# jmhb0/view_neti

Hardware: AMD Instinct MI355X
Metric: TI train steps/sec (SD-1.5 512^2 bs=4 per GPU) (higher is better)
Workload: dtype f16; 1 GPU; learnable_mode 0, sd15 shapes, 512x512 fp16, bs=4/GPU, grad_accum 1, full train step (VAE+16xCLIP+UNet fwd/bwd+AdamW); global_batch=4, parallelism=dp1, rccl_ranks=1, hipgraph=True

## Files before the change

### include/vneti.h

```cpp
#ifndef VNETI_H
#define VNETI_H
#include <stddef.h>
#include <stdint.h>

#ifdef __cplusplus
extern "C" {
#endif

#define VNETI_ABI_VERSION 1

int vneti_version(void);
int vneti_precision(void);
int vneti_last_error(char* buf, size_t n);

typedef struct vneti_gemm_desc {
  const void* A;
  const void* B;
  void* C;
  long long lda, ldb, ldc;
  int M, N, K;
  int batch;
  long long strideA, strideB, strideC;
  const float* bias;
  const void* rowadd;
  long long ld_rowadd;
  int rows_per_group;
  const void* resid;
  long long ldr;
  float alpha;
  int act;
  int out_f32;
  int conv_mode;
  int Hi, Wi, Ci, Ho, Wo, stride, pad_t, pad_l, ups;
  long long ldx;
  int tile_hint;
  void* workspace;
  long long workspace_bytes;
  int split_k;
  const void* gate_src;
  long long ld_gate;
  int gate_act;
  void* C2;
  long long ldc2;
  int act2;
  void* gn_sums;
  int gn_hw, gn_cpg, gn_groups, gn_slots;
  int geglu;
  int conv_korder;
} vneti_gemm_desc;

int vneti_gemm_f16(const vneti_gemm_desc* d, void* stream);
int vneti_gemm_select_tile(int M, int N, int batch);
int vneti_gemm_select_split(int M, int N, int K, int batch, int tile_hint, long long workspace_bytes);

int vneti_im2col3x3_small(const void* x, int x_is_f32, long long sb, long long sc, long long sy,
                          long long sx, void* out, int Bn, int C, int Hi, int Wi, int Ho, int Wo,
                          int stride, int pad_t, int pad_l, void* stream);

int vneti_conv3x3_in(const void* x, int x_is_f32, long long sb, long long sc, long long sy, long long sx,
                     const void* w_packed, const float* bias, void* out, long long ldo, int Bn, int C, int H, int W,
                     int Co, void* gn_sums, int gn_groups, int gn_slots, void* stream);

int vneti_transpose_f16(const void* in, long long ld_in, long long stride_in, void* out,
                        long long ld_out, long long stride_out, int rows, int cols, int batch,
                        void* stream);
#define VNETI_TRANSPOSE_MAX 4
typedef struct vneti_transpose_desc {
  const void* inp;
  long long ld_in, stride_in;
  void* out;
  long long ld_out, stride_out;
  int rows, cols, batch, _pad;
} vneti_transpose_desc;
int vneti_transpose_f16_multi(const vneti_transpose_desc* descs, int n, void* stream);

long long vneti_groupnorm_ws_floats(int Bn, int HW, int C, int G);
int vneti_groupnorm_fwd(const void* x, long long ldx, void* y, long long ldy, const float* gamma,
                        const float* beta, float* mean, float* rstd, float* ws, int Bn, int HW,
                        int C, int G, float eps, int silu, void* stream);
int vneti_groupnorm_fwd_sums(const void* x, long long ldx, void* y, long long ldy, const float* gamma,
                             const float* beta, const void* sums, int slots, float* mean, float* rstd,
                             int Bn, int HW, int C, int G, float eps, int silu, void* stream);
int vneti_groupnorm_fwd_2l(const void* x, long long ldx, void* y, long long ldy, const float* gamma,
                           const float* beta, void* sums, int slots, float* mean, float* rstd, int Bn, int HW,
                           int C, int G, float eps, int silu, void* stream);
int vneti_groupnorm_bwd_2l(const void* dy, long long lddy, const void* x, long long ldx, const float* gamma,
                           const float* beta, const float* mean, const float* rstd, void* dx, long long lddx,
                           const void* dx_accum, long long ldacc, void* sums, int slots, float* ws, int Bn,
                           int HW, int C, int G, int silu, void* stream);
int vneti_groupnorm_bwd(const void* dy, long long lddy, const void* x, long long ldx,
                        const float* gamma, const float* beta, const float* mean,
                        const float* rstd, void* dx, long long lddx, const void* dx_accum,
                        long long ldacc, float* ws, int Bn, int HW, int C, int G, int silu,
                        void* stream);

int vneti_layernorm_fwd(const void* x, int x_is_f32, long long ldx, void* y, long long ldy,
                        const float* gamma, const float* beta, float* mean, float* rstd, int rows,
                        int C, float eps, void* stream);
int vneti_layernorm_bwd(const void* dy, int dy_is_f32, long long lddy, const void* x,
                        int x_is_f32, long long ldx, const float* gamma, const float* mean,
                        const float* rstd, void* dx, int dx_is_f32, long long lddx,
                        const void* dx_accum, long long ldacc, void* dx_f16_copy, long long ldcopy,
                        int rows, int C, void* stream);

int vneti_attn_fwd(const void* Q, long long ldq, const void* K, long long ldk, const void* V,
                   long long ldv, void* O, long long ldo, float* lse, int Bn, int H, int Nq,
// ... 159 lines not shown
```

### view_neti_amd/csrc/gemm_conv.hip

```cpp
#include "common.h"
#include "gemm_args.h"
#include "../../include/vneti.h"

namespace {

template <int BM, int BN, int WM, int WN, bool F32OUT, bool DMA, int NSTG = 2, int EPI = 2, bool CONV = true>
__global__ __launch_bounds__((BM / WM) * (BN / WN) * 64) void gemm_kernel(
    const half_t* pA, const half_t* pB, uint32_t p_a_bytes, uint32_t p_b_bytes, int p_lda, int p_ldb, int pM, int pN, int pK,
    int p_tiles_m, int p_tiles_n, int p_split_conv , const GemmArgs gfull) {
  GemmArgs g = gfull;
  g.A = pA;
  g.B = pB;
  g.a_bytes = p_a_bytes;
  g.b_bytes = p_b_bytes;
  g.lda = p_lda;
  g.ldb = p_ldb;
  g.M = pM;
  g.N = pN;
  g.K = pK;
  g.tiles_m = p_tiles_m;
  g.tiles_n = p_tiles_n;
  g.kt_per_split = p_split_conv & 0xffff;
  g.ksplit = (p_split_conv >> 16) & 0xff;
  g.conv_mode = p_split_conv >> 24;
  static_assert(NSTG == 2 || ((NSTG == 3 || NSTG == 4) && DMA), "the LDS rings are LDS-DMA only");
  const half_t* const e_gate = EPI == 2 ? g.gate_src : nullptr;
  half_t* const e_C2 = EPI == 2 ? g.C2 : nullptr;
  const int e_geglu = EPI == 2 ? g.geglu : 0;
  const int e_act = EPI == 2 ? g.act : 0;
  float* const e_gn_sums = EPI >= 1 ? g.gn_sums : nullptr;
  const half_t* const e_rowadd = EPI >= 1 ? g.rowadd : nullptr;
  const int e_conv = CONV ? g.conv_mode : 0;
  constexpr int NWM = BM / WM, NWN = BN / WN;
  constexpr int NT = NWM * NWN * 64;
  constexpr int RSTEP = NT / 8;
  constexpr int A_IT = BM / RSTEP, B_IT = BN / RSTEP;
  constexpr int STAGE_BYTES = (BM + BN) * 128;
  constexpr int CS_LD = F32OUT ? (BN + 4) : (BN + 8);
  constexpr int CS_BYTES = BM * CS_LD * (F32OUT ? 4 : 2);
  constexpr int LDS_BYTES = (NSTG * STAGE_BYTES > CS_BYTES) ? NSTG * STAGE_BYTES : CS_BYTES;
  constexpr int GN_IMG = 5, GN_NG = BN / 4 + 2;
  constexpr int GN_BYTES = (F32OUT || EPI == 0) ? 0 : GN_IMG * GN_NG * 4 * 8;
  __shared__ __attribute__((aligned(16))) char smem[LDS_BYTES + GN_BYTES];

  const int tid = threadIdx.x;
  const int lane = tid & 63;
  const int wave = __builtin_amdgcn_readfirstlane(tid >> 6);
  const int wm0 = (wave / NWN) * WM;
  const int wn0 = (wave % NWN) * WN;

  int nblk = g.tiles_m * g.tiles_n;
  int bid = blockIdx.x;
  {
    int q = nblk >> 3, r = nblk & 7, xcd = bid & 7, idx = bid >> 3;
    bid = (xcd < r ? xcd * (q + 1) : r * (q + 1) + (xcd - r) * q) + idx;
  }
  const int tile_m = bid / g.tiles_n;
  const int tile_n = bid - tile_m * g.tiles_n;
  const int m0 = tile_m * BM;
  const int n0 = tile_n * BN;
  const int bz = blockIdx.y;
  const int kz = blockIdx.z;

  const half_t* Ab = g.A + (long long)bz * g.strideA;
  const half_t* Bb = g.B + (long long)bz * g.strideB;
  __amdgpu_buffer_rsrc_t rsA = vn_make_rsrc(Ab, g.a_bytes);
  __amdgpu_buffer_rsrc_t rsB = vn_make_rsrc(Bb, g.b_bytes);

  const int lrow = tid >> 3;
  const int gchunk = DMA ? ((tid & 7) ^ ((lrow >> 1) & 7)) : (tid & 7);

  const float rcp_hw = CONV ? __builtin_amdgcn_rcpf((float)(g.Ho * g.Wo)) : 0.f, rcp_wo = CONV ? __builtin_amdgcn_rcpf((float)g.Wo) : 0.f;
  int a_off[A_IT];
  int a_py[A_IT], a_px[A_IT], a_bh[A_IT];
#pragma unroll
  for (int i = 0; i < A_IT; ++i) {
    int m = m0 + lrow + RSTEP * i;
    bool ok = m < g.M;
    if (e_conv == 0) {
      a_off[i] = ok ? (int)((long long)m * g.lda * 2) + gchunk * 16 : -1;
      a_py[i] = a_px[i] = a_bh[i] = 0;
    } else {
      int rem, ox;
      const int b = vn_divmod(m, g.Ho * g.Wo, rcp_hw, rem);
      const int oy = vn_divmod(rem, g.Wo, rcp_wo, ox);
      a_bh[i] = ok ? b * g.Hi : -1;
      if (e_conv == 1) {
        a_py[i] = oy * g.stride - g.pad_t;
        a_px[i] = ox * g.stride - g.pad_l;
      } else {
        a_py[i] = oy + g.pad_t;
        a_px[i] = ox + g.pad_l;
      }
      a_off[i] = ((b * g.Hi + a_py[i]) * g.Wi + a_px[i]) * g.ldx2 + gchunk * 16;
    }
  }
  int b_off[B_IT];
#pragma unroll
  for (int i = 0; i < B_IT; ++i) {
    int n = n0 + lrow + RSTEP * i;
    b_off[i] = (n < g.N) ? (int)((long long)n * g.ldb * 2) + gchunk * 16 : -1;
  }

  u32x4 ra[DMA ? 1 : A_IT], rb[DMA ? 1 : B_IT];

  auto a_offset = [&](int i, int k0, int dy, int dx, int tapoff) -> uint32_t {
    if (e_conv == 0) return a_off[i] < 0 ? VN_OOB : (uint32_t)(a_off[i] + k0 * 2);
    bool ok = a_bh[i] >= 0;
    if (e_conv == 1 && !g.ups) {
      int iy = a_py[i] + dy, ix = a_px[i] + dx;
      ok = ok && (unsigned)iy < (unsigned)g.Hi && (unsigned)ix < (unsigned)g.Wi;
      return ok ? (uint32_t)(a_off[i] + tapoff) : VN_OOB;
    }
    int iy, ix;
    if (e_conv == 1) {
// ... 765 lines not shown
  if (cfg == 17 && f32) cfg = 7;
  if ((cfg == 6 || cfg == 7) && !dma) cfg = 4;
  if (cfg >= 10 && !dma) cfg = kTiles[cfg].bm == 128 ? (kTiles[cfg].bn == 128 ? 1 : 2) : 3;
  long long ws_floats = d->workspace ? d->workspace_bytes / 4 : 0;
  int ks = d->split_k;
  if (ks == 0) ks = select_ksplit(d->M, d->N, d->K, batch, cfg, ws_floats);
  if (ks < 1) ks = 1;
  const int nk = d->K / 64;
  if (ks > nk) ks = nk;
  if (ks > 1) {
    VN_REQUIRE(d->workspace && (long long)ks * batch * d->M * d->N <= ws_floats,
               "gemm: split_k=%d needs %lld workspace bytes", ks, (long long)ks * batch * d->M * d->N * 4);
    VN_REQUIRE(batch == 1 || (d->strideC != 0), "gemm: batched split-K needs strideC");
    VN_REQUIRE((long long)batch * d->M * ((d->N + 3) / 4) < 0x7fffffffLL, "gemm: split-K output larger than 2^31 chunks");
    VN_REQUIRE_OUT("gemm split-K workspace", (long long)ks * batch * d->M * d->N * 4);
  }
  if (cfg == 18 && ks > d->Ci / 64) ks = d->Ci / 64;
  g.ksplit = ks;
  g.kt_per_split = cdiv(nk, ks);
  g.ksplit = cdiv(nk, g.kt_per_split);
  VN_REQUIRE(g.ksplit <= 255 && g.kt_per_split <= 0xffff, "gemm: split_k=%d / K=%d out of range", g.ksplit, d->K);
  g.ws = (float*)d->workspace;

#define LAUNCH(BM, BN, WM, WN) \
  return dma ? launch_cfg<BM, BN, WM, WN, true>(g, f32, st) : launch_cfg<BM, BN, WM, WN, false>(g, f32, st)
  switch (cfg) {
    case 1: LAUNCH(128, 128, 64, 64);
    case 2: LAUNCH(128, 64, 64, 32);
    case 3: LAUNCH(64, 64, 32, 32);
    case 4: LAUNCH(256, 128, 64, 64);
    case 6: return launch_cfg_ring<256, 128, 64, 64>(g, f32, st);
    case 7: return launch_cfg_ring<256, 128, 64, 32>(g, f32, st);
    case 8: LAUNCH(256, 128, 64, 32);
    case 9: LAUNCH(128, 128, 64, 32);
    case 10: return launch_cfg_ring<128, 128, 64, 32>(g, f32, st);
    case 11: return launch_cfg_ring<128, 64, 64, 32>(g, f32, st);
    case 12: return launch_cfg_ring<64, 64, 32, 32>(g, f32, st);
    case 13: return launch_cfg_ring<128, 128, 64, 32, 4>(g, f32, st);
    case 14: return launch_cfg_ring<128, 64, 64, 32, 4>(g, f32, st);
    case 15: return launch_cfg_ring<64, 64, 32, 32, 4>(g, f32, st);
    case 16:
    case 17:
    case 18: {
      const int rc = vneti_launch_gemm8(&g, cfg == 16 ? 256 : 128, cfg == 18 ? 1 : 0, st);
      if (rc != VNETI_OK) return rc;
      launch_reduce(g, st);
      return vneti_check_launch("gemm8_kernel");
    }
    default:
      return dma ? launch_cfg_f16<256, 256, 64, 64, true>(g, st) : launch_cfg_f16<256, 256, 64, 64, false>(g, st);
  }
#undef LAUNCH
}
```

### view_neti_amd/engine/step.py

```python
from __future__ import annotations

from functools import partial
from typing import Dict, List, Optional

import torch

from .. import ops
from .. import sd_config as sc
from .graphs import capture_graphs
from .text import MapperState, TextEngine
from .unet import UNetEngine
from .vae import VAEEncoderEngine


def alphas_cumprod(cfg: sc.DDPMConfig) -> torch.Tensor:
    betas = torch.linspace(cfg.beta_start ** 0.5, cfg.beta_end ** 0.5, cfg.num_train_timesteps,
                           dtype=torch.float32) ** 2
    return torch.cumprod(1.0 - betas, dim=0)


class TrainStepEngine:
    def __init__(self, cfg: sc.SDConfig, unet_w: Dict, vae_w: Dict, clip_w: Dict, batch: int, height: int,
                 width: int, mapper_object: Dict[str, torch.Tensor], w_enc_object: torch.Tensor,
                 norm_scale_object: Optional[float], alpha_object: float = 0.2,
                 mapper_view: Optional[Dict[str, torch.Tensor]] = None, w_enc_view: Optional[torch.Tensor] = None,
                 norm_scale_view: Optional[float] = None, alpha_view: float = 0.2, train_view: bool = True,
                 n_view_params: int = 12, lr: float = 1e-3, betas=(0.9, 0.999), adam_eps: float = 1e-8,
                 weight_decay: float = 1e-2, loss_scale: Optional[float] = None, growth_interval: int = 2000,
                 seed: int = 0, world_size: int = 1, device_rng: bool = True, device: str = "cuda",
                 need_backward: bool = True, grad_accum: int = 1, overlap: bool = False,
                 unconstrained_object: bool = False, unconstrained_view: bool = False,
                 nested_dropout_prob: float = 0.0, hidden_object: int = 64,
                 legacy_pe_object: Optional[torch.Tensor] = None, enc_dim_object: int = 64,
                 output_bypass_object: bool = True, output_bypass_view: bool = True, exchange=None,
                 moment_cache_images: int = 0):
        from .text import flatten_mapper_state
        self.cfg = cfg
        self.B, self.H, self.W = batch, height, width
        self.dev = device
        self.world_size = world_size
        self.exchange = exchange
        if world_size > 1 and exchange is None:
            import os
            import torch.distributed as dist
            if os.environ.get("VNETI_RCCL_DIRECT", "1") != "0" and dist.is_initialized() and dist.get_backend() == "nccl":
                from ..parallel import enable_direct_rccl
                try:
                    self.exchange = enable_direct_rccl()
                except RuntimeError as err:
                    if os.environ.get("VNETI_REQUIRE_ONE_GRAPH", "0") == "1":
                        raise
                    import warnings
                    warnings.warn(f"library RCCL communicator unavailable ({err}); using torch.distributed.all_reduce")
        self.device_rng = device_rng
        if loss_scale is None:
            from .. import lib
            loss_scale = 1.0 if lib.precision() == "bf16" else 65536.0
            if lib.precision() == "bf16":
                growth_interval = 0
        self.growth_interval = growth_interval
        nlev = len(cfg.vae.block_out_channels)
        self.h, self.w = height >> (nlev - 1), width >> (nlev - 1)
        Lc = cfg.vae.latent_channels
        D = cfg.clip.hidden_size
        objs = list(mapper_object) if isinstance(mapper_object, (list, tuple)) else [mapper_object]
        flats = [flatten_mapper_state(sd) for sd in objs]
        self.n_objects = len(flats)
        self.n_obj = flats[0].numel()
        assert all(f.numel() == self.n_obj for f in flats), "object mappers must share one architecture"
        flat_v = flatten_mapper_state(mapper_view) if (mapper_view is not None and train_view) else None
        n_all_obj = self.n_obj * self.n_objects
        n = n_all_obj + (flat_v.numel() if flat_v is not None else 0)
        self.params = torch.zeros(n, dtype=torch.float32, device=device)
        self.params[:n_all_obj].copy_(torch.cat(flats))
        if flat_v is not None:
            self.params[n_all_obj:].copy_(flat_v)
        self.grads = torch.zeros_like(self.params)
        self.exp_avg = torch.zeros_like(self.params)
        self.exp_avg_sq = torch.zeros_like(self.params)
        self.n_all_obj = n_all_obj
        self.obj_slot = torch.zeros(1, dtype=torch.int32, device=device)
        self.seg_step = torch.zeros(self.n_objects, dtype=torch.int32, device=device)
        self.active_object = 0
        multi = self.n_objects > 1
        self.rng_state = torch.tensor([seed & 0x7FFFFFFF, 0], dtype=torch.int32, device=device)
        mo = MapperState(self.params[:n_all_obj],
                         w_enc_object.to(device).float().contiguous() if legacy_pe_object is None else None,
                         norm_scale_object, alpha_object, hidden=hidden_object, enc_dim=enc_dim_object,
                         unconstrained=unconstrained_object,
                         nested_dropout_prob=nested_dropout_prob, slot=self.obj_slot if multi else None,
                         slot_stride=self.n_obj if multi else 0,
                         legacy_w_pe=(legacy_pe_object.to(device).float().contiguous()
                                      if legacy_pe_object is not None else None),
                         output_bypass=output_bypass_object)
        mv, gv = None, None
        if mapper_view is not None:
            if flat_v is not None:
                pv, gv = self.params[n_all_obj:], self.grads[n_all_obj:]
            else:
                pv = flatten_mapper_state(mapper_view).to(device)
            mv = MapperState(pv, w_enc_view.to(device).float().contiguous(), norm_scale_view, alpha_view,
                             unconstrained=unconstrained_view,
                             nested_dropout_prob=nested_dropout_prob if flat_v is not None else 0.0,
                             output_bypass=output_bypass_view)
        self.grad_accum = grad_accum
        self.hyper = torch.tensor([lr, betas[0], betas[1], adam_eps, weight_decay, float(world_size * grad_accum)],
                                  dtype=torch.float32, device=device)
        self.scaler = torch.tensor([loss_scale, 0.0, 0.0], dtype=torch.float32, device=device)
        self.opt_step = torch.zeros(1, dtype=torch.int32, device=device)
        self.loss_sum = torch.zeros(1, dtype=torch.float32, device=device)
        self.ac = alphas_cumprod(cfg.ddpm).to(device)
        from ..parallel import shared_picks
        with shared_picks():
            self.unet = UNetEngine(cfg.unet, unet_w, batch, self.h, self.w, cfg.clip.max_positions, device, need_backward)
            self.vae = VAEEncoderEngine(cfg.vae, vae_w, batch, height, width, device)
            self.text = TextEngine(cfg.clip, clip_w, cfg.unet.n_cross_layers, batch, self.unet.timesteps, self.unet.ctx_k,
                                   self.unet.ctx_v, self.unet.dctx_k, self.unet.dctx_v, mo, self.grads[:n_all_obj], mv,
                                   gv, n_view_params, train_view, device, need_backward, rng_state=self.rng_state)
        self.timesteps = self.unet.timesteps
        self.pixel_values = self.vae.x_in
        shape = (batch, Lc, self.h, self.w)
        self.eps = torch.zeros(shape, dtype=torch.float32, device=device)
        self.noise = torch.zeros(shape, dtype=torch.float32, device=device)
        self.latents = torch.zeros(shape, dtype=torch.float32, device=device)
        self.target = torch.zeros(shape, dtype=torch.float32, device=device)
        self.n_cache = int(moment_cache_images)
        if self.n_cache:
            hw2 = self.h * self.w
            self.mcache = torch.zeros(self.n_cache, hw2, 2 * Lc, dtype=self.vae.moments.dtype, device=device)
            self.img_idx = torch.zeros(batch, dtype=torch.int64, device=device)
            self._cached_images = set()
            self._batch_cached = False
            self._batch_images = ()
        self.graph_a_c = self.graph_acc_c = None
        self.eval_out = torch.zeros(batch, dtype=torch.float32, device=device)
        self.eval_ws = torch.zeros(ops.mse_loss_per_sample_ws_floats(batch, self.h * self.w), dtype=torch.float32,
                                   device=device)
        self.graph_eval = None
        from .staging import HostStager
        self.stager = HostStager()
        self.need_backward = need_backward
        self.overlap = overlap
        self.side = torch.cuda.Stream() if overlap else None
        self.graph_a = self.graph_b = self.graph_acc = None
        self.exchange_in_graph = False
        self._reduce_stage = None
        self.last_reduce_bytes = 0
        self.micro = 0
        self._eval_batch = False
        self.n_loss = batch * Lc * self.h * self.w

    def set_batch(self, pixel_values, input_ids, placeholder_object, placeholder_view=None, view_params=None,
                  object_index: int = 0, image_idx=None, for_eval: bool = False):
        if not 0 <= object_index < self.n_objects:
            raise ValueError(f"object_index {object_index} out of range (have {self.n_objects} object mappers)")
        if self.micro != 0 and object_index != self.active_object:
            raise ValueError("the object mapper may not change inside a gradient-accumulation group")
        self.active_object = object_index
        self.obj_slot.fill_(object_index)
        self._eval_batch = bool(for_eval)
        st = self.stager
        st.begin()
        try:
            if self.n_cache and for_eval:
                self._batch_images, self._batch_cached = (), False
            elif self.n_cache:
                if image_idx is None:
# ... 297 lines not shown
```

### view_neti_amd/engine/unet.py

```python
from __future__ import annotations

from functools import partial
from typing import Dict

import torch

from .. import ops, packing
from .. import sd_config as sc
from .schedule import Schedule, T, rup as _rup


class UNetEngine(Schedule):
    def __init__(self, cfg: sc.UNetConfig, weights: Dict[str, torch.Tensor], batch: int, height: int, width: int,
                 ctx_len: int = 77, device: str = "cuda", need_backward: bool = True, autotune: bool = True,
                 fuse_gn: bool = True):
        super().__init__(batch, cfg.norm_num_groups, cfg.norm_eps, device, need_backward)
        self.cfg = cfg
        self.H, self.W = height, width
        self.L = ctx_len
        self.nl = cfg.n_cross_layers
        B, L, Dc = batch, ctx_len, cfg.cross_attention_dim
        self.x_in = self._buf((B, cfg.in_channels, height, width), torch.float32)
        self.timesteps = torch.zeros(B, dtype=torch.int64, device=device)
        self.ctx_k = self._buf((self.nl, B * L, Dc))
        self.ctx_v = self._buf((self.nl, B * L, Dc))
        self.dctx_k = self._buf((self.nl, B * L, Dc))
        self.dctx_v = self._buf((self.nl, B * L, Dc))
        self.pred = self._buf((B * height * width, 8))[:, : cfg.out_channels]
        self.dpred = self._buf((B * height * width, 8), zero=True)[:, : cfg.out_channels]
        self._pack_time_weights(weights)
        self._plan_kv()
        self._build(weights)
        self._kv_fwd_ops()
        if need_backward:
            self._build_backward()
            self._kv_bwd_ops()
        if autotune:
            self.autotune()
        self.bind_workspace()
        self.fuse_gn_stats(fuse=fuse_gn)

    def _pack_time_weights(self, w):
        cfg = self.cfg
        names = [k[: -len("time_emb_proj.weight")] for k in sc.unet_shapes(cfg) if k.endswith("time_emb_proj.weight")]
        self.temb_off = {}
        ws, bs, off = [], [], 0
        for n in names:
            wt = w[n + "time_emb_proj.weight"]
            self.temb_off[n] = (off, wt.shape[0])
            ws.append(wt)
            bs.append(w[n + "time_emb_proj.bias"])
            off += wt.shape[0]
        self.temb_total = off
        self.w_temb_all = self._w16(torch.cat(ws, 0))
        self.b_temb_all = self._w32(torch.cat(bs, 0))
        self.w_t1 = self._w16(w["time_embedding.linear_1.weight"])
        self.b_t1 = self._w32(w["time_embedding.linear_1.bias"])
        self.w_t2 = self._w16(w["time_embedding.linear_2.weight"])
        self.b_t2 = self._w32(w["time_embedding.linear_2.bias"])
        c0, td = cfg.block_out_channels[0], cfg.temb_dim
        self.t_sin = self._buf((self.B, c0))
        self.t_h = self._buf((self.B, td))
        self.t_emb = self._buf((self.B, td))
        self.temb_all = self._buf((self.B, self.temb_total))

    def _time_ops(self):
        f = self.fwd_pre
        f.append(partial(ops.timestep_embedding, self.timesteps, self.t_sin))
        f.append(partial(ops.gemm, self.t_sin, self.w_t1, self.t_h, bias=self.b_t1, act=ops.ACT_SILU, tile_hint=3))
        f.append(partial(ops.gemm, self.t_h, self.w_t2, self.t_emb, bias=self.b_t2, act=ops.ACT_SILU, tile_hint=3))
        f.append(partial(ops.gemm, self.t_emb, self.w_temb_all, self.temb_all, bias=self.b_temb_all, tile_hint=3))

    def _cross_widths(self):
        cfg = self.cfg
        boc, lpb = cfg.block_out_channels, cfg.layers_per_block
        ws = []
        for i, a in enumerate(cfg.down_has_attn):
            ws += [boc[i]] * lpb if a else []
        ws.append(boc[-1])
        for i, a in enumerate(reversed(cfg.down_has_attn)):
            ws += [tuple(reversed(boc))[i]] * (lpb + 1) if a else []
        assert len(ws) == self.nl
        return ws

    def _plan_kv(self):
        B, L, Dc = self.B, self.L, self.cfg.cross_attention_dim
        ws = self._cross_widths()
        self.kv_runs, self.kv_slot = [], {}
        l0 = 0
        while l0 < len(ws):
            n = 1
            while l0 + n < len(ws) and ws[l0 + n] == ws[l0]:
                n += 1
            Cc = ws[l0]
            run = dict(l0=l0, n=n, C=Cc, wk=self._buf((n, Cc, Dc)), wv=self._buf((n, Cc, Dc)),
                       k=self._buf((n, B * L, Cc)), v=self._buf((n, B * L, Cc)))
            if self.need_backward:
                run.update(wkd=self._buf((n, Dc, Cc)), wvd=self._buf((n, Dc, Cc)),
                           dk=self._buf((n, B * L, Cc)), dv=self._buf((n, B * L, Cc)))
            for j in range(n):
                self.kv_slot[l0 + j] = (run, j)
            self.kv_runs.append(run)
            l0 += n

    def _kv_fwd_ops(self):
        B, L, Dc = self.B, self.L, self.cfg.cross_attention_dim
        for run in self.kv_runs:
            l0, n, Cc = run["l0"], run["n"], run["C"]
            for ctx, wgt, out in ((self.ctx_k, run["wk"], run["k"]), (self.ctx_v, run["wv"], run["v"])):
                self.fwd_pre.append(partial(ops.gemm, ctx[l0], wgt[0], out[0], batch=n, strideA=B * L * Dc,
                                            strideB=Cc * Dc, strideC=B * L * Cc))

    def _kv_bwd_ops(self):
        B, L, Dc = self.B, self.L, self.cfg.cross_attention_dim
        for run in self.kv_runs:
            l0, n, Cc = run["l0"], run["n"], run["C"]
            for dsrc, wgt, dctx in ((run["dk"], run["wkd"], self.dctx_k), (run["dv"], run["wvd"], self.dctx_v)):
                self.bwd.append(partial(ops.gemm, dsrc[0], wgt[0], dctx[l0], batch=n, strideA=B * L * Cc,
                                        strideB=Dc * Cc, strideC=B * L * Dc))

    def _transformer(self, x: T, Cc, heads, name, w, layer_idx, out_view, h, wd, need_dx=True):
        cfg = self.cfg
        B, L, Dc = self.B, self.L, cfg.cross_attention_dim
        M, N = x.rows, h * wd
        D = Cc // heads
        scale = D ** -0.5
        t = name + "transformer_blocks.0."
        r = dict(kind="transformer", x=x, C=Cc, heads=heads, D=D, N=N, name=name, layer=layer_idx, need_dx=need_dx,
                 scale=scale)
        g, r["gn"] = self._gn(x, name + "norm", w, 1e-6, False)
        w_in = w[name + "proj_in.weight"].reshape(Cc, Cc)
        r["w_in"], b_in = self._w16(w_in), self._w32(w[name + "proj_in.bias"])
        h0 = self._buf((M, Cc))
        self.fwd.append(partial(ops.gemm, g, r["w_in"], h0, bias=b_in))
        n1, r["ln1"] = self._ln(h0, t + "norm1", w)
        wqkv = torch.cat([w[t + "attn1.to_q.weight"], w[t + "attn1.to_k.weight"], w[t + "attn1.to_v.weight"]], 0)
        r["wqkv"] = self._w16(wqkv)
        qkv = self._buf((M, 3 * Cc))
        self.fwd.append(partial(ops.gemm, n1, r["wqkv"], qkv))
        q, k, v = qkv[:, :Cc], qkv[:, Cc:2 * Cc], qkv[:, 2 * Cc:]
        o1 = self._buf((M, Cc))
        lse1 = self._buf((B, heads, N), torch.float32)
        self.fwd.append(partial(ops.attn_fwd, q, k, v, o1, lse1, B, heads, N, N, D, scale, False))
        r["wo1"], bo1 = self._w16(w[t + "attn1.to_out.0.weight"]), self._w32(w[t + "attn1.to_out.0.bias"])
        h1 = self._buf((M, Cc))
        self.fwd.append(partial(ops.gemm, o1, r["wo1"], h1, bias=bo1, resid=h0))
        n2, r["ln2"] = self._ln(h1, t + "norm2", w)
        r["wq2"] = self._w16(w[t + "attn2.to_q.weight"])
        run, slot = self.kv_slot[layer_idx]
        assert run["C"] == Cc, (name, layer_idx, Cc, run["C"])
        run["wk"][slot].copy_(w[t + "attn2.to_k.weight"])
        run["wv"][slot].copy_(w[t + "attn2.to_v.weight"])
        q2 = self._buf((M, Cc))
        k2, v2 = run["k"][slot], run["v"][slot]
        self.fwd.append(partial(ops.gemm, n2, r["wq2"], q2))
        o2 = self._buf((M, Cc))
        lse2 = self._buf((B, heads, N), torch.float32)
        self.fwd.append(partial(ops.attn_fwd, q2, k2, v2, o2, lse2, B, heads, N, L, D, scale, False))
        r["wo2"], bo2 = self._w16(w[t + "attn2.to_out.0.weight"]), self._w32(w[t + "attn2.to_out.0.bias"])
        h2 = self._buf((M, Cc))
        self.fwd.append(partial(ops.gemm, o2, r["wo2"], h2, bias=bo2, resid=h1))
        n3, r["ln3"] = self._ln(h2, t + "norm3", w)
        wff1_il = packing.geglu_interleave(w[t + "ff.net.0.proj.weight"])
        r["wff1"], bff1 = self._w16(wff1_il), self._w32(packing.geglu_interleave(w[t + "ff.net.0.proj.bias"]))
        r["wff2"], bff2 = self._w16(w[t + "ff.net.2.weight"]), self._w32(w[t + "ff.net.2.bias"])
        p = self._buf((M, 8 * Cc))
        gg = self._buf((M, 4 * Cc))
        self.fwd.append(partial(ops.gemm, n3, r["wff1"], p, bias=bff1, out2=gg, geglu=1, split_k=1))
        h3 = self._buf((M, Cc))
        self.fwd.append(partial(ops.gemm, gg, r["wff2"], h3, bias=bff2, resid=h2))
        r["w_out"], b_out = self._w16(w[name + "proj_out.weight"].reshape(Cc, Cc)), self._w32(w[name + "proj_out.bias"])
        out = T(out_view if out_view is not None else self._buf((M, Cc)))
# ... 236 lines not shown
```

### view_neti_amd/lib.py

```python
from __future__ import annotations

import ctypes as C
import keyword
import os
import re

_HERE = os.path.dirname(os.path.abspath(__file__))
HEADER_PATH = os.path.join(os.path.dirname(_HERE), "include", "vneti.h")

_PRECISIONS = {"fp16": ("libvneti_hip.so", 0), "bf16": ("libvneti_hip_bf16.so", 1)}
_precision = os.environ.get("VNETI_PRECISION", "fp16")
if _precision not in _PRECISIONS:
    raise RuntimeError(f"VNETI_PRECISION={_precision!r}: expected one of {sorted(_PRECISIONS)}")

_lib = None


def so_path(precision: str = None) -> str:
    return os.environ.get("VNETI_LIB_PATH") or os.path.join(_HERE, "csrc", _PRECISIONS[precision or _precision][0])


SO_PATH = so_path()


# ... 27 lines not shown
        return _SCALARS[base]
    if stars == 1 and base == "char":
        return C.c_char_p
    if stars == 1 and base in structs:
        return C.POINTER(structs[base])
    if stars and (base in _SCALARS or base in ("void", "char")):
        return C.c_void_p
    raise ValueError(f"vneti.h {where}: no ctypes rule for the type {ctype.strip()!r}")


def _declarator(decl: str, where: str):
    m = re.fullmatch(r"(.*[\s*])(\w+)", decl.strip(), re.S)
    if not m:
        raise ValueError(f"vneti.h {where}: cannot read the declaration {' '.join(decl.split())!r}")
    return m.group(1), m.group(2)


def parse_header(text: str):
    blank = lambda m: "\n" * m.group().count("\n")
    text = re.sub(r"/\*.*?\*/|//[^\n]*", blank, text, flags=re.S)
    text = re.sub(r'^[ \t]*#.*$|extern\s+"C"\s*\{|^\}[ \t]*$', "", text, flags=re.M)
    at = lambda src, pos: f"line {src.count(chr(10), 0, pos) + 1}"
    structs, protos = {}, {}
    typedef = r"typedef\s+struct\s+\w*\s*\{(.*?)\}\s*(\w+)\s*;"
    for m in re.finditer(typedef, text, flags=re.S):
        fields = []
        for d in re.finditer(r"[^;\s][^;]*", m.group(1)):
            where = at(text, m.start(1) + d.start())
            first, *more = d.group().split(",")
            ctype, name = _declarator(first, where)
            for n in [name] + [x.strip() for x in more]:
                if not n.isidentifier() or keyword.iskeyword(n):
                    raise ValueError(f"vneti.h {where}: cannot bind the field {n!r}")
                fields.append((n, _ctype(ctype, structs, where)))
        structs[m.group(2)] = type(m.group(2), (C.Structure,), {"_fields_": fields})
    rest = re.sub(typedef, blank, text, flags=re.S)
    for m in re.finditer(r"[^;\s][^;]*", rest):
        p = re.fullmatch(r"(int|long long)\s+(vneti_\w+)\s*\((.*)\)\s*", m.group(), re.S)
        if not p:
            raise ValueError(f"vneti.h {at(rest, m.start())}: cannot read {' '.join(m.group().split())!r} as a prototype")
        argtypes = []
        for x in re.finditer(r"[^,\s][^,]*", "" if p.group(3).strip() == "void" else p.group(3)):
            where = at(rest, m.start() + p.start(3) + x.start())
            argtypes.append(_ctype(_declarator(x.group(), where)[0], structs, where))
        protos[p.group(2)] = (_SCALARS[p.group(1)], argtypes)
    return structs, protos


with open(HEADER_PATH) as _f:
    _STRUCTS, _PROTOS = parse_header(_f.read())
GemmDesc, TransposeDesc = _STRUCTS["vneti_gemm_desc"], _STRUCTS["vneti_transpose_desc"]
SIGNATURES = {n[len("vneti_"):]: argtypes for n, (_, argtypes) in _PROTOS.items()}
VALUE_FUNCS = frozenset({
    "version", "precision", "last_error", "gemm_select_tile", "gemm_select_split", "img_resample_ksize",
    "groupnorm_ws_floats", "lpips_ws_floats", "mse_loss_per_sample_ws_floats", "mapper_num_params", "mapper_save_floats",
    "mapper_rowgrad_floats", "mapper_legacy_input_params"})
_stray = ({n[len("vneti_"):] for n, (res, _) in _PROTOS.items() if res is C.c_longlong} - VALUE_FUNCS) | (VALUE_FUNCS - set(SIGNATURES))
if _stray:
    raise RuntimeError(f"lib.VALUE_FUNCS is out of step with include/vneti.h: {sorted(_stray)}")


def declared_symbols() -> list[str]:
    src = open(HEADER_PATH).read()
    src = re.sub(r"/\*.*?\*/", "", src, flags=re.S)
    return sorted(set(re.findall(r"\b(vneti_[a-z0-9_]+)\s*\(", src)))


def load():
    global _lib
    if _lib is not None:
        return _lib
    if not os.path.exists(SO_PATH):
        raise RuntimeError(
            f"{os.path.basename(SO_PATH)} not found at {SO_PATH}: build it with "
            "`python view_neti_amd/csrc/build.py` (hipcc, gfx950). There is no fallback path.")
    lib = C.CDLL(SO_PATH)
    for name, (restype, argtypes) in _PROTOS.items():
        fn = getattr(lib, name, None)
        if fn is None:
            raise RuntimeError(f"{SO_PATH} does not export {name}, which include/vneti.h declares: rebuild it")
        fn.restype, fn.argtypes = restype, argtypes
    if lib.vneti_precision() != _PRECISIONS[_precision][1]:
        raise RuntimeError(f"{SO_PATH} computes in precision {lib.vneti_precision()}, the process asked for {_precision}")
    _lib = lib
    return lib


def last_error() -> str:
    lib = load()
    buf = C.create_string_buffer(512)
    lib.vneti_last_error(buf, 512)
    return buf.value.decode(errors="replace")


def check(rc: int, what: str = ""):
    if rc != 0:
        raise RuntimeError(f"vneti call failed ({what}) rc={rc}: {last_error()}")


def call(name: str, *args):
    check(getattr(load(), "vneti_" + name)(*args), name)


def query(name: str, *args) -> int:
    if name not in VALUE_FUNCS:
        raise KeyError(f"vneti_{name} returns a status: use call()")
    return int(getattr(load(), "vneti_" + name)(*args))
# ... 1 lines not shown
```

### view_neti_amd/ops.py

```python
from __future__ import annotations

import ctypes as C

import torch

from . import lib as _l

ACT_NONE, ACT_SILU, ACT_QUICK_GELU, ACT_GELU = 0, 1, 2, 3


def stream() -> int:
    return torch.cuda.current_stream().cuda_stream


def _p(t):
    return None if t is None else t.data_ptr()


def _ld(t):
    if t is None:
        return 0
    assert t.stride(-1) == 1, "last dim must be contiguous"
    return t.stride(-2) if t.dim() >= 2 else t.shape[-1]


_default_ws = None


def set_default_gemm_workspace(t):
    global _default_ws
    _default_ws = t


def gemm(A, B, out, *, bias=None, rowadd=None, rows_per_group=1, resid=None, alpha=1.0, act=0,
         tile_hint=0, batch=0, strideA=0, strideB=0, strideC=0, M=None, N=None, K=None, conv=None,
         lda=None, ldc=None, workspace=None, split_k=0, gate=None, gate_act=0, out2=None, act2=0,
         gn_sums=None, gn_hw=0, gn_groups=0, gn_slots=0, geglu=0):
    d = _l.GemmDesc()
    d.A, d.B, d.C = _p(A), _p(B), _p(out)
    d.ldb = _ld(B)
    d.ldc = ldc if ldc is not None else _ld(out)
    d.N = N if N is not None else B.shape[-2]
    d.K = K if K is not None else B.shape[-1]
    if conv is None:
        d.M = M if M is not None else A.shape[-2]
        d.lda = lda if lda is not None else _ld(A)
        d.conv_mode = 0
    else:
        d.M = M
        d.lda = 0
        d.conv_mode = conv["mode"]
        for k in ("Hi", "Wi", "Ci", "Ho", "Wo", "stride", "pad_t", "pad_l", "ups", "ldx"):
            setattr(d, k, int(conv.get(k, 0)))
        d.conv_korder = int(conv.get("korder", 0))
    d.batch = batch
    d.strideA, d.strideB, d.strideC = strideA, strideB, strideC
    d.bias = _p(bias)
    d.rowadd = _p(rowadd)
    d.ld_rowadd = _ld(rowadd) if rowadd is not None else 0
    d.rows_per_group = rows_per_group
    d.resid = _p(resid)
    d.ldr = _ld(resid) if resid is not None else 0
    d.alpha = alpha
    d.act = act
    d.out_f32 = 1 if out.dtype == torch.float32 else 0
    d.tile_hint = tile_hint
    if gate is not None:
        d.gate_src, d.ld_gate, d.gate_act = _p(gate), _ld(gate), gate_act
    if out2 is not None:
        d.C2, d.ldc2, d.act2 = _p(out2), _ld(out2), act2
    if gn_sums is not None:
        d.gn_sums, d.gn_hw, d.gn_groups, d.gn_slots = _p(gn_sums), gn_hw, gn_groups, gn_slots
        d.gn_cpg = d.N // gn_groups
    d.geglu = geglu
    ws = workspace if workspace is not None else _default_ws
    if ws is not None:
        d.workspace = ws.data_ptr()
        d.workspace_bytes = ws.numel() * ws.element_size()
    d.split_k = split_k if ws is not None else 1
    _l.call("gemm_f16", C.byref(d), stream())


def im2col3x3_small(x, out, Bn, Cc, Hi, Wi, Ho, Wo, stride, pad_t, pad_l, strides):
    sb, sc, sy, sx = strides
    _l.call("im2col3x3_small", _p(x), 1 if x.dtype == torch.float32 else 0, sb, sc, sy, sx, _p(out),
            Bn, Cc, Hi, Wi, Ho, Wo, stride, pad_t, pad_l, stream())


def conv3x3_in(x, w_packed, bias, out, Bn, Cc, H, W, strides, gn_sums=None, gn_hw=0, gn_groups=0, gn_slots=0):
    sb, sc, sy, sx = strides
    assert gn_sums is None or gn_hw == H * W
    _l.call("conv3x3_in", _p(x), 1 if x.dtype == torch.float32 else 0, sb, sc, sy, sx, _p(w_packed), _p(bias), _p(out),
            _ld(out), Bn, Cc, H, W, w_packed.shape[0], _p(gn_sums), gn_groups, gn_slots, stream())


def transpose(inp, out, rows, cols, batch, ld_in, stride_in, ld_out, stride_out):
    _l.call("transpose_f16", _p(inp), ld_in, stride_in, _p(out), ld_out, stride_out, rows, cols, batch, stream())


def transpose_multi(items):
    arr = (_l.TransposeDesc * len(items))()
    for d, (inp, out, rows, cols, batch, ld_in, stride_in, ld_out, stride_out) in zip(arr, items):
        d.inp, d.ld_in, d.stride_in = _p(inp), ld_in, stride_in
        d.out, d.ld_out, d.stride_out = _p(out), ld_out, stride_out
        d.rows, d.cols, d.batch = rows, cols, batch
    _l.call("transpose_f16_multi", arr, len(items), stream())


def groupnorm_ws_floats(Bn, HW, Cc, G):
    n = _l.query("groupnorm_ws_floats", Bn, HW, Cc, G)
    if n < 0:
        raise RuntimeError(f"groupnorm: unsupported shape {(Bn, HW, Cc, G)}")
    return n


def groupnorm_fwd(x, y, gamma, beta, mean, rstd, ws, Bn, HW, Cc, G, eps, silu):
    _l.call("groupnorm_fwd", _p(x), _ld(x), _p(y), _ld(y), _p(gamma), _p(beta), _p(mean), _p(rstd), _p(ws),
            Bn, HW, Cc, G, eps, 1 if silu else 0, stream())


def groupnorm_fwd_sums(x, y, gamma, beta, sums, slots, mean, rstd, Bn, HW, Cc, G, eps, silu):
    _l.call("groupnorm_fwd_sums", _p(x), _ld(x), _p(y), _ld(y), _p(gamma), _p(beta), _p(sums), slots, _p(mean), _p(rstd),
            Bn, HW, Cc, G, eps, 1 if silu else 0, stream())


def groupnorm_fwd_2l(x, y, gamma, beta, sums, slots, mean, rstd, Bn, HW, Cc, G, eps, silu):
    _l.call("groupnorm_fwd_2l", _p(x), _ld(x), _p(y), _ld(y), _p(gamma), _p(beta), _p(sums), slots, _p(mean), _p(rstd),
            Bn, HW, Cc, G, eps, 1 if silu else 0, stream())


def groupnorm_bwd_2l(dy, x, gamma, beta, mean, rstd, dx, sums, slots, ws, Bn, HW, Cc, G, silu, accum=None):
    _l.call("groupnorm_bwd_2l", _p(dy), _ld(dy), _p(x), _ld(x), _p(gamma), _p(beta), _p(mean), _p(rstd),
            _p(dx), _ld(dx), _p(accum), _ld(accum) if accum is not None else 0, _p(sums), slots, _p(ws),
# ... 367 lines not shown
```

### view_neti_amd/roofline.py

```python
from __future__ import annotations

import torch

from . import ops

import os as _os

_CSRC = _os.path.join(_os.path.dirname(_os.path.abspath(__file__)), "csrc")
MFMA_PEAK_TFLOPS = 2500.0
HBM_PEAK_TBS = 8.0
PF, TB = MFMA_PEAK_TFLOPS, HBM_PEAK_TBS


def kernel_tree_sha() -> str:
    import hashlib
    import os
    here = _CSRC
    files = sorted(os.path.join(here, f) for f in os.listdir(here) if f.endswith((".hip", ".h")))
    files.append(os.path.join(os.path.dirname(os.path.dirname(here)), "include", "vneti.h"))
    h = hashlib.sha256()
    for f in files:
        h.update(os.path.basename(f).encode())
        h.update(open(f, "rb").read())
    return h.hexdigest()[:16]


def gemm_cost(f):
    kw = f.keywords
    A, Bm = f.args[0], f.args[1]
    M = kw.get("M") or A.shape[-2]
    N, K = kw.get("N") or Bm.shape[-2], kw.get("K") or Bm.shape[-1]
    batch = kw.get("batch") or 1
    conv = kw.get("conv")
    a_bytes = (M // (conv["Ho"] * conv["Wo"])) * conv["Hi"] * conv["Wi"] * conv["Ci"] * 2 if conv else M * K * 2 * batch
    out = f.args[2]
    c_cols = N * (2 if kw.get("geglu") == 2 else 1)
    extra = sum(M * c * 2 for c, key in ((N, "resid"), (N, "out2"), (c_cols, "gate")) if kw.get(key) is not None)
    if kw.get("geglu") == 1:
        extra -= M * N
    nbytes = a_bytes + N * K * 2 * batch + M * c_cols * out.element_size() * batch + extra
    flops = 2.0 * M * N * K * batch
    return M, N, K, batch, flops, nbytes, flops / (MFMA_PEAK_TFLOPS * 1e12), nbytes / (HBM_PEAK_TBS * 1e12)



def cost(f):
    fn, a, kw = getattr(f, "func", None), getattr(f, "args", ()), getattr(f, "keywords", {}) or {}
    if fn is ops.gemm:
        M, N, K, batch, flops, nbytes, t_mfma, t_hbm = gemm_cost(f)
        if t_hbm > t_mfma:
            return ("gemm, below the ridge (short-K linears: HBM-bound)", 0, nbytes)
        return ("gemm / implicit-GEMM conv (MFMA-bound)", flops, 0)
    if fn in (ops.attn_fwd, ops.attn_bwd_dq, ops.attn_bwd_dkv):
        i = {ops.attn_fwd: 5, ops.attn_bwd_dq: 7, ops.attn_bwd_dkv: 8}[fn]
        Bn, H, Nq, Nk, D = a[i:i + 5]
        causal = a[i + 6]
        mm = {ops.attn_fwd: 2, ops.attn_bwd_dq: 3, ops.attn_bwd_dkv: 4}[fn]
        name = {ops.attn_fwd: "attention fwd", ops.attn_bwd_dq: "attention bwd dQ", ops.attn_bwd_dkv: "attention bwd dK/dV"}[fn]
        scores = Bn * H * Nq * Nk * (0.5 if causal else 1.0)
        ks, db = -(-D // 16), -(-D // 32)
        mfma_c = {ops.attn_fwd: ks + 2 * db, ops.attn_bwd_dq: 2 * ks + 2 * db, ops.attn_bwd_dkv: 2 * ks + 4 * db}[fn] * 32 / 1024.0
        valu_c = {ops.attn_fwd: 2.8, ops.attn_bwd_dq: 4.0, ops.attn_bwd_dkv: 4.0}[fn] * 2 / 64.0 + (2 * 5 / 3) / 64.0
        cob = scores * (mfma_c + valu_c) / (1024 * 2.4e9)
        return (name, mm * 2.0 * scores * D, 0, cob)
    if fn is ops.attn_bwd_small:
        Bn, H, N, D = a[9:13]
        return ("attention bwd (short sequences, one launch)", 7 * 2.0 * Bn * H * N * N * D * (0.5 if a[14] else 1.0), 0)
    if fn in (ops.groupnorm_fwd, ops.groupnorm_fwd_sums, ops.groupnorm_fwd_2l):
        Bn, HW, C = (a[7], a[8], a[9]) if fn is ops.groupnorm_fwd else (a[8], a[9], a[10])
        return ("GroupNorm(+SiLU) fwd" + (" (stats in producer)" if fn is ops.groupnorm_fwd_sums else ""), 0, 2.0 * Bn * HW * C * 2)
    if fn is ops.layernorm_fwd:
        x, y = a[0], a[1]
        return ("LayerNorm fwd", 0, x.numel() * x.element_size() + y.numel() * y.element_size())
    if getattr(f, "vn_cost", None) is not None:
        return (f.vn_cost[0], 0, f.vn_cost[1])
    if getattr(fn, "__name__", "") == "_ln_bwd":
        x = a[0]["x"]
        n = x.numel()
        extra = (a[3].numel() * a[3].element_size() if a[3] is not None else 0) + (n * 2 if len(a) > 4 and a[4] is not None else 0)
        return ("LayerNorm bwd", 0, n * x.element_size() + a[1].numel() * a[1].element_size() + a[2].numel() * a[2].element_size() + extra)
    if fn in (ops.groupnorm_bwd, ops.groupnorm_bwd_2l):
        x = a[1]
        return ("GroupNorm(+SiLU) bwd", 0, 5.0 * x.numel() * 2)
    if fn is ops.add:
        return ("elementwise glue (add, 2x2 sum, transposes, noise, loss)", 0, sum(t.numel() * t.element_size() for t in a[:3]))
    if fn is ops.sum2x2:
        return ("elementwise glue (add, 2x2 sum, transposes, noise, loss)", 0, a[0].numel() * 2 + a[1].numel() * 2)
    if fn in (ops.sample_add_noise, ops.mse_loss_grad, getattr(ops, "transpose", None), getattr(ops, "timestep_embedding", None)):
        return ("elementwise glue (add, 2x2 sum, transposes, noise, loss)", 0,
                sum(t.numel() * t.element_size() for t in a if isinstance(t, torch.Tensor)))
    if fn is ops.layernorm_bwd:
        return ("LayerNorm bwd", 0, sum(t.numel() * t.element_size() for t in (a[0], a[1], a[5])))
    if fn is ops.conv3x3_in:
        return ("VAE conv_in (direct)", 0, a[0].numel() * 4 + a[3].numel() * 2)
    if fn is ops.softmax_rows:
        return ("softmax rows (VAE mid attention)", 0, 2.0 * a[0].numel() * 2)
    if fn is ops.geglu_fwd:
        return ("GEGLU fwd", 0, a[0].numel() * 2 + a[1].numel() * 2)
    if fn is ops.geglu_bwd:
        return ("GEGLU bwd", 0, a[0].numel() * 2 + 2 * a[1].numel() * 2)
    return None


# ... 53 lines not shown
```

Before: 39.55 steps/s.

## Group cross-attention K/V projection GEMMs into one grouped kernel launch per tile

Adds a grouped GEMM path in which each block reads its own GemmArgs from a device-side table indexed by blockIdx.y. The UNet engine uses it to collapse the per-run batched K/V context projection GEMMs, forward and backward, into one launch per tile configuration. The aim is to cut launch count and tail underuse from many small GEMMs in the graph. Grouped launches size grid.x to the widest group, so narrower groups exit early, and groups needing split-K fall back to the old path.

```diff
diff --git a/include/vneti.h b/include/vneti.h
--- a/include/vneti.h
+++ b/include/vneti.h
@@ -52,6 +52,10 @@
 int vneti_gemm_f16(const vneti_gemm_desc* d, void* stream);
 int vneti_gemm_select_tile(int M, int N, int batch);
 int vneti_gemm_select_split(int M, int N, int K, int batch, int tile_hint, long long workspace_bytes);
+
+long long vneti_gemm_grouped_table_bytes(int n);
+int vneti_gemm_grouped_pack(const vneti_gemm_desc* descs, int n, void* table_host, int* grid_x);
+int vneti_gemm_grouped_f16(const void* table, int n, int grid_x, int tile_hint, void* stream);
 
 int vneti_im2col3x3_small(const void* x, int x_is_f32, long long sb, long long sc, long long sy,
                           long long sx, void* out, int Bn, int C, int Hi, int Wi, int Ho, int Wo,
diff --git a/view_neti_amd/csrc/gemm_conv.hip b/view_neti_amd/csrc/gemm_conv.hip
--- a/view_neti_amd/csrc/gemm_conv.hip
+++ b/view_neti_amd/csrc/gemm_conv.hip
@@ -4,25 +4,31 @@
 
 namespace {
 
-template <int BM, int BN, int WM, int WN, bool F32OUT, bool DMA, int NSTG = 2, int EPI = 2, bool CONV = true>
+template <int BM, int BN, int WM, int WN, bool F32OUT, bool DMA, int NSTG = 2, int EPI = 2, bool CONV = true, bool GROUPED = false>
 __global__ __launch_bounds__((BM / WM) * (BN / WN) * 64) void gemm_kernel(
     const half_t* pA, const half_t* pB, uint32_t p_a_bytes, uint32_t p_b_bytes, int p_lda, int p_ldb, int pM, int pN, int pK,
     int p_tiles_m, int p_tiles_n, int p_split_conv , const GemmArgs gfull) {
   GemmArgs g = gfull;
-  g.A = pA;
-  g.B = pB;
-  g.a_bytes = p_a_bytes;
-  g.b_bytes = p_b_bytes;
-  g.lda = p_lda;
-  g.ldb = p_ldb;
-  g.M = pM;
-  g.N = pN;
-  g.K = pK;
-  g.tiles_m = p_tiles_m;
-  g.tiles_n = p_tiles_n;
-  g.kt_per_split = p_split_conv & 0xffff;
-  g.ksplit = (p_split_conv >> 16) & 0xff;
-  g.conv_mode = p_split_conv >> 24;
+  if constexpr (GROUPED) {
+    static_assert(!F32OUT && !CONV && EPI == 0, "grouped launches: plain f16 GEMMs with the level-0 epilogue");
+    g = reinterpret_cast<const GemmArgs*>(pA)[blockIdx.y];
+    if ((int)blockIdx.x >= g.tiles_m * g.tiles_n) return;
+  } else {
+    g.A = pA;
+    g.B = pB;
+    g.a_bytes = p_a_bytes;
+    g.b_bytes = p_b_bytes;
+    g.lda = p_lda;
+    g.ldb = p_ldb;
+    g.M = pM;
+    g.N = pN;
+    g.K = pK;
+    g.tiles_m = p_tiles_m;
+    g.tiles_n = p_tiles_n;
+    g.kt_per_split = p_split_conv & 0xffff;
+    g.ksplit = (p_split_conv >> 16) & 0xff;
+    g.conv_mode = p_split_conv >> 24;
+  }
   static_assert(NSTG == 2 || ((NSTG == 3 || NSTG == 4) && DMA), "the LDS rings are LDS-DMA only");
   const half_t* const e_gate = EPI == 2 ? g.gate_src : nullptr;
   half_t* const e_C2 = EPI == 2 ? g.C2 : nullptr;
@@ -59,8 +65,8 @@
   const int tile_n = bid - tile_m * g.tiles_n;
   const int m0 = tile_m * BM;
   const int n0 = tile_n * BN;
-  const int bz = blockIdx.y;
-  const int kz = blockIdx.z;
+  const int bz = GROUPED ? 0 : blockIdx.y;
+  const int kz = GROUPED ? 0 : blockIdx.z;
 
   const half_t* Ab = g.A + (long long)bz * g.strideA;
   const half_t* Bb = g.B + (long long)bz * g.strideB;
@@ -932,3 +938,84 @@
   }
 #undef LAUNCH
 }
+
+namespace {
+
+inline bool grouped_tile_ok(int tile) { return tile == 3 || tile == 13 || tile == 14 || tile == 15; }
+
+template <int BM, int BN, int WM, int WN, int NSTG>
+int launch_grouped(const void* table, int n, int grid_x, hipStream_t st) {
+  const dim3 grid(grid_x, n, 1), block((BM / WM) * (BN / WN) * 64);
+  GemmArgs none;
+  memset(&none, 0, sizeof(none));
+  hipLaunchKernelGGL((gemm_kernel<BM, BN, WM, WN, false, true, NSTG, 0, false, true>), grid, block, 0, st, (const half_t*)table,
+                     (const half_t*)nullptr, 0u, 0u, 0, 0, 0, 0, 0, 0, 0, 0, none);
+  return vneti_check_launch("gemm_kernel (grouped)");
+}
+
+}
+
+extern "C" long long vneti_gemm_grouped_table_bytes(int n) { return n > 0 ? (long long)n * (long long)sizeof(GemmArgs) : -1; }
+
+extern "C" int vneti_gemm_grouped_pack(const vneti_gemm_desc* descs, int n, void* table_host, int* grid_x) {
+  VN_REQUIRE(descs != nullptr && table_host != nullptr && grid_x != nullptr, "gemm grouped: null argument");
+  VN_REQUIRE(n >= 1 && n <= 65535, "gemm grouped: %d groups (1 .. 65535: grid.y)", n);
+  const int tile = descs[0].tile_hint;
+  VN_REQUIRE(grouped_tile_ok(tile), "gemm grouped: tile_hint %d has no grouped form (3, 13, 14, 15)", tile);
+  GemmArgs* tab = (GemmArgs*)table_host;
+  int widest = 0;
+  for (int i = 0; i < n; ++i) {
+    const vneti_gemm_desc* d = descs + i;
+    VN_REQUIRE(d->A && d->B && d->C, "gemm grouped: group %d: null operand pointer", i);
+    VN_REQUIRE(d->M > 0 && d->N > 0 && d->K > 0 && d->K % 64 == 0, "gemm grouped: group %d: bad shape M=%d N=%d K=%d", i, d->M,
+               d->N, d->K);
+    VN_REQUIRE(d->lda % 8 == 0 && d->ldb % 8 == 0 && (d->ldc % 8 == 0 || d->N < 8), "gemm grouped: group %d: lda / ldb / ldc %% 8", i);
+    VN_REQUIRE(d->tile_hint == tile, "gemm grouped: group %d is pinned to tile %d, the launch to %d", i, d->tile_hint, tile);
+    VN_REQUIRE(d->conv_mode == 0, "gemm grouped: group %d is an implicit convolution", i);
+    VN_REQUIRE(d->split_k == 1, "gemm grouped: group %d: split_k=%d (must be 1)", i, d->split_k);
+    VN_REQUIRE(!d->out_f32, "gemm grouped: group %d: f32 output", i);
+    VN_REQUIRE(d->batch <= 1, "gemm grouped: group %d: batch=%d (one group per matrix)", i, d->batch);
+    VN_REQUIRE(!d->rowadd && !d->resid && !d->gate_src && !d->C2 && !d->gn_sums && !d->geglu && !d->act,
+               "gemm grouped: group %d carries an epilogue operand (bias only)", i);
+    const long long a_bytes = ((long long)(d->M - 1) * d->lda + d->K) * 2, b_bytes = ((long long)(d->N - 1) * d->ldb + d->K) * 2;
+    VN_REQUIRE(a_bytes < 0x7fffffffLL && b_bytes < 0x7fffffffLL, "gemm grouped: group %d: operand larger than 2 GiB", i);
+    VN_REQUIRE_OUT("gemm grouped C", vn_out_bytes(d->M, d->ldc, d->N, 2));
+    GemmArgs& g = tab[i];
+    memset(&g, 0, sizeof(g));
+    g.A = (const half_t*)d->A;
+    g.B = (const half_t*)d->B;
+    g.C = d->C;
+    g.bias = d->bias;
+    g.lda = d->lda;
+    g.ldb = d->ldb;
+    g.ldc = d->ldc;
+    g.a_bytes = (uint32_t)a_bytes;
+    g.b_bytes = (uint32_t)b_bytes;
+    g.M = d->M;
+    g.N = d->N;
+    g.K = d->K;
+    g.rows_per_group = 1;
+    g.alpha = d->alpha;
+    g.batch = 1;
+    g.ksplit = 1;
+    g.kt_per_split = d->K / 64;
+    g.tiles_m = cdiv(d->M, kTiles[tile].bm);
+    g.tiles_n = cdiv(d->N, kTiles[tile].bn);
+    if (g.tiles_m * g.tiles_n > widest) widest = g.tiles_m * g.tiles_n;
+  }
+  *grid_x = widest;
+  return VNETI_OK;
+}
+
+extern "C" int vneti_gemm_grouped_f16(const void* table, int n, int grid_x, int tile_hint, void* stream) {
+  VN_REQUIRE(table != nullptr, "gemm grouped: null table");
+  VN_REQUIRE(n >= 1 && n <= 65535 && grid_x >= 1, "gemm grouped: bad grid %d x %d", grid_x, n);
+  VN_REQUIRE(grouped_tile_ok(tile_hint), "gemm grouped: tile_hint %d has no grouped form (3, 13, 14, 15)", tile_hint);
+  hipStream_t st = (hipStream_t)stream;
+  switch (tile_hint) {
+    case 3: return launch_grouped<64, 64, 32, 32, 2>(table, n, grid_x, st);
+    case 13: return launch_grouped<128, 128, 64, 32, 4>(table, n, grid_x, st);
+    case 14: return launch_grouped<128, 64, 64, 32, 4>(table, n, grid_x, st);
+    default: return launch_grouped<64, 64, 32, 32, 4>(table, n, grid_x, st);
+  }
+}
diff --git a/view_neti_amd/engine/step.py b/view_neti_amd/engine/step.py
--- a/view_neti_amd/engine/step.py
+++ b/view_neti_amd/engine/step.py
@@ -33,7 +33,7 @@
                  nested_dropout_prob: float = 0.0, hidden_object: int = 64,
                  legacy_pe_object: Optional[torch.Tensor] = None, enc_dim_object: int = 64,
                  output_bypass_object: bool = True, output_bypass_view: bool = True, exchange=None,
-                 moment_cache_images: int = 0):
+                 moment_cache_images: int = 0, group_launches: bool = True):
         from .text import flatten_mapper_state
         self.cfg = cfg
         self.B, self.H, self.W = batch, height, width
@@ -112,7 +112,8 @@
         self.ac = alphas_cumprod(cfg.ddpm).to(device)
         from ..parallel import shared_picks
         with shared_picks():
-            self.unet = UNetEngine(cfg.unet, unet_w, batch, self.h, self.w, cfg.clip.max_positions, device, need_backward)
+            self.unet = UNetEngine(cfg.unet, unet_w, batch, self.h, self.w, cfg.clip.max_positions, device, need_backward,
+                                   group_kv=group_launches)
             self.vae = VAEEncoderEngine(cfg.vae, vae_w, batch, height, width, device)
             self.text = TextEngine(cfg.clip, clip_w, cfg.unet.n_cross_layers, batch, self.unet.timesteps, self.unet.ctx_k,
                                    self.unet.ctx_v, self.unet.dctx_k, self.unet.dctx_v, mo, self.grads[:n_all_obj], mv,
diff --git a/view_neti_amd/engine/unet.py b/view_neti_amd/engine/unet.py
--- a/view_neti_amd/engine/unet.py
+++ b/view_neti_amd/engine/unet.py
@@ -13,7 +13,7 @@
 class UNetEngine(Schedule):
     def __init__(self, cfg: sc.UNetConfig, weights: Dict[str, torch.Tensor], batch: int, height: int, width: int,
                  ctx_len: int = 77, device: str = "cuda", need_backward: bool = True, autotune: bool = True,
-                 fuse_gn: bool = True):
+                 fuse_gn: bool = True, group_kv: bool = True):
         super().__init__(batch, cfg.norm_num_groups, cfg.norm_eps, device, need_backward)
         self.cfg = cfg
         self.H, self.W = height, width
@@ -38,6 +38,8 @@
         if autotune:
             self.autotune()
         self.bind_workspace()
+        if group_kv:
+            self._group_kv()
         self.fuse_gn_stats(fuse=fuse_gn)
 
     def _pack_time_weights(self, w):
@@ -105,6 +107,7 @@
 
     def _kv_fwd_ops(self):
         B, L, Dc = self.B, self.L, self.cfg.cross_attention_dim
+        self._kv_fwd_at = len(self.fwd_pre)
         for run in self.kv_runs:
             l0, n, Cc = run["l0"], run["n"], run["C"]
             for ctx, wgt, out in ((self.ctx_k, run["wk"], run["k"]), (self.ctx_v, run["wv"], run["v"])):
@@ -113,11 +116,40 @@
 
     def _kv_bwd_ops(self):
         B, L, Dc = self.B, self.L, self.cfg.cross_attention_dim
+        self._kv_bwd_at = len(self.bwd)
         for run in self.kv_runs:
             l0, n, Cc = run["l0"], run["n"], run["C"]
             for dsrc, wgt, dctx in ((run["dk"], run["wkd"], self.dctx_k), (run["dv"], run["wvd"], self.dctx_v)):
                 self.bwd.append(partial(ops.gemm, dsrc[0], wgt[0], dctx[l0], batch=n, strideA=B * L * Cc,
                                         strideB=Dc * Cc, strideC=B * L * Dc))
+
+    def _group_kv(self):
+        nkv = 2 * len(self.kv_runs)
+        for lst, at in ((self.fwd_pre, self._kv_fwd_at),) + (((self.bwd, self._kv_bwd_at),) if self.need_backward else ()):
+            by_tile, keep = {}, []
+            for f in lst[at:at + nkv]:
+                kw = dict(f.keywords)
+                n, sA, sB, sC = kw.pop("batch"), kw.pop("strideA"), kw.pop("strideB"), kw.pop("strideC")
+                A, Bm, out = f.args
+                tile = kw.get("tile_hint") or ops.gemm_select_tile(A.shape[-2], Bm.shape[-2], n)
+                ws = kw.get("workspace")
+                split = kw.get("split_k", 0) if ws is not None else 1
+                if split == 0:
+                    split = ops.gemm_select_split(A.shape[-2], Bm.shape[-2], Bm.shape[-1], n, tile,
+                                                  ws.numel() * ws.element_size())
+                if tile not in (3, 13, 14, 15) or split != 1:
+                    keep.append(f)
+                    continue
+                el = lambda t, stride, j: t.as_strided(t.shape, t.stride(), t.storage_offset() + j * stride)
+                by_tile.setdefault(tile, []).extend(
+                    dict(kw, A=el(A, sA, j), B=el(Bm, sB, j), out=el(out, sC, j), tile_hint=tile, split_k=1) for j in range(n))
+            grouped = []
+            for tile, groups in by_tile.items():
+                table, n, grid_x, tile = ops.gemm_grouped_pack(groups, self.dev)
+                self.bytes += table.numel()
+                grouped.append(partial(ops.gemm_grouped, table, n, grid_x, tile,
+                                       shapes=tuple((g["A"].shape[-2], g["B"].shape[-2], g["B"].shape[-1]) for g in groups)))
+            lst[at:at + nkv] = grouped + keep
 
     def _transformer(self, x: T, Cc, heads, name, w, layer_idx, out_view, h, wd, need_dx=True):
         cfg = self.cfg
diff --git a/view_neti_amd/lib.py b/view_neti_amd/lib.py
--- a/view_neti_amd/lib.py
+++ b/view_neti_amd/lib.py
@@ -103,7 +103,8 @@
 GemmDesc, TransposeDesc = _STRUCTS["vneti_gemm_desc"], _STRUCTS["vneti_transpose_desc"]
 SIGNATURES = {n[len("vneti_"):]: argtypes for n, (_, argtypes) in _PROTOS.items()}
 VALUE_FUNCS = frozenset({
-    "version", "precision", "last_error", "gemm_select_tile", "gemm_select_split", "img_resample_ksize",
+    "version", "precision", "last_error", "gemm_select_tile", "gemm_select_split", "gemm_grouped_table_bytes",
+    "img_resample_ksize",
     "groupnorm_ws_floats", "lpips_ws_floats", "mse_loss_per_sample_ws_floats", "mapper_num_params", "mapper_save_floats",
     "mapper_rowgrad_floats", "mapper_legacy_input_params"})
 _stray = ({n[len("vneti_"):] for n, (res, _) in _PROTOS.items() if res is C.c_longlong} - VALUE_FUNCS) | (VALUE_FUNCS - set(SIGNATURES))
diff --git a/view_neti_amd/ops.py b/view_neti_amd/ops.py
--- a/view_neti_amd/ops.py
+++ b/view_neti_amd/ops.py
@@ -36,6 +36,17 @@
          tile_hint=0, batch=0, strideA=0, strideB=0, strideC=0, M=None, N=None, K=None, conv=None,
          lda=None, ldc=None, workspace=None, split_k=0, gate=None, gate_act=0, out2=None, act2=0,
          gn_sums=None, gn_hw=0, gn_groups=0, gn_slots=0, geglu=0):
+    d = _gemm_desc(A, B, out, bias=bias, rowadd=rowadd, rows_per_group=rows_per_group, resid=resid, alpha=alpha, act=act,
+                   tile_hint=tile_hint, batch=batch, strideA=strideA, strideB=strideB, strideC=strideC, M=M, N=N, K=K,
+                   conv=conv, lda=lda, ldc=ldc, workspace=workspace, split_k=split_k, gate=gate, gate_act=gate_act, out2=out2,
+                   act2=act2, gn_sums=gn_sums, gn_hw=gn_hw, gn_groups=gn_groups, gn_slots=gn_slots, geglu=geglu)
+    _l.call("gemm_f16", C.byref(d), stream())
+
+
+def _gemm_desc(A, B, out, *, bias=None, rowadd=None, rows_per_group=1, resid=None, alpha=1.0, act=0,
+               tile_hint=0, batch=0, strideA=0, strideB=0, strideC=0, M=None, N=None, K=None, conv=None,
+               lda=None, ldc=None, workspace=None, split_k=0, gate=None, gate_act=0, out2=None, act2=0,
+               gn_sums=None, gn_hw=0, gn_groups=0, gn_slots=0, geglu=0):
     d = _l.GemmDesc()
     d.A, d.B, d.C = _p(A), _p(B), _p(out)
     d.ldb = _ld(B)
@@ -78,7 +89,26 @@
         d.workspace = ws.data_ptr()
         d.workspace_bytes = ws.numel() * ws.element_size()
     d.split_k = split_k if ws is not None else 1
-    _l.call("gemm_f16", C.byref(d), stream())
+    return d
+
+
+def gemm_grouped_pack(groups, device):
+    n = len(groups)
+    arr = (_l.GemmDesc * n)()
+    for i, kw in enumerate(groups):
+        kw = dict(kw)
+        d = _gemm_desc(kw.pop("A"), kw.pop("B"), kw.pop("out"), **kw)
+        if d.split_k == 0 and not d.conv_mode:
+            d.split_k = _l.query("gemm_select_split", d.M, d.N, d.K, max(d.batch, 1), d.tile_hint, d.workspace_bytes)
+        C.memmove(C.addressof(arr[i]), C.addressof(d), C.sizeof(d))
+    host = torch.zeros(_l.query("gemm_grouped_table_bytes", n), dtype=torch.uint8)
+    grid_x = C.c_int(0)
+    _l.call("gemm_grouped_pack", arr, n, host.data_ptr(), C.byref(grid_x))
+    return host.to(device), n, grid_x.value, arr[0].tile_hint
+
+
+def gemm_grouped(table, n, grid_x, tile_hint, shapes=None):
+    _l.call("gemm_grouped_f16", table.data_ptr(), n, grid_x, tile_hint, stream())
 
 
 def im2col3x3_small(x, out, Bn, Cc, Hi, Wi, Ho, Wo, stride, pad_t, pad_l, strides):
diff --git a/view_neti_amd/roofline.py b/view_neti_amd/roofline.py
--- a/view_neti_amd/roofline.py
+++ b/view_neti_amd/roofline.py
@@ -49,6 +49,13 @@
     if fn is ops.gemm:
         M, N, K, batch, flops, nbytes, t_mfma, t_hbm = gemm_cost(f)
         if t_hbm > t_mfma:
+            return ("gemm, below the ridge (short-K linears: HBM-bound)", 0, nbytes)
+        return ("gemm / implicit-GEMM conv (MFMA-bound)", flops, 0)
+    if fn is ops.gemm_grouped:
+        shapes = kw.get("shapes") or ()
+        flops = sum(2.0 * M * N * K for M, N, K in shapes)
+        nbytes = sum((M * K + N * K + M * N) * 2 for M, N, K in shapes)
+        if nbytes / (HBM_PEAK_TBS * 1e12) > flops / (MFMA_PEAK_TFLOPS * 1e12):
             return ("gemm, below the ridge (short-K linears: HBM-bound)", 0, nbytes)
         return ("gemm / implicit-GEMM conv (MFMA-bound)", flops, 0)
     if fn in (ops.attn_fwd, ops.attn_bwd_dq, ops.attn_bwd_dkv):
```

After: 39.64 steps/s, median of 5. About the same (+0.2%).
